# JiapengWu/TeMP

Measured on AMD Instinct MI355X. Metric: edges/sec (fwd+bwd) RGCN+GRU seq_len=15, higher is better.
Workload: dtype f32

## Files before the change

temp_amd/csrc/gemm_hx.hpp:

```cpp
#pragma once
#include "gemm_bx.hpp"
#include "hx_pack.hpp"

namespace temp {

struct HxPacked { const hx_u32x4* b[PANEL_MAXP]; const unsigned* keys[PANEL_MAXP]; };

template <int G, class Epi>
__global__ void __launch_bounds__(BX_THREADS, (G <= 4 ? 3 : 2)) k_gemm_hxp(PanelBatch<Epi> batch, BxGeom g, HxPacked packed, int keys_by_out) {
  constexpr int PIECES = G * 128;
  constexpr int NPC = (PIECES + BX_THREADS - 1) / BX_THREADS;
  __shared__ __attribute__((aligned(16))) hx_u32x4 Bs[2][PIECES];
  const PanelProblem<Epi>& pb = batch.p[blockIdx.y];
  const int M = pb.M;
  const int xcd = blockIdx.x & 7, local = blockIdx.x >> 3;
  const int grp = local % g.n_groups, rt_local = local / g.n_groups;
  const int rt = xcd * g.per_xcd + rt_local;
  if (rt_local >= g.per_xcd || rt * 128 >= M) return;
  const bool tail = grp == g.n_groups - 1;
  const int t0 = tail ? g.n_tiles - G : grp * G;
  const int t_store = tail ? G - g.tail_store : 0;
  const int n0 = t0 * 32;
  const int N = g.N, K = g.K;
  const float* __restrict__ A = pb.A;
  const int32_t* __restrict__ a_idx = pb.a_idx;
  const Epi& epi = pb.epi;
  const int lane = threadIdx.x & 63, wave = threadIdx.x >> 6;
  const int hh = lane >> 5, li = lane & 31;
  const int row = rt * 128 + wave * 32 + li;
  long a_src = -1;
  if (row < M) a_src = a_idx ? (long)a_idx[row] : (long)row;
  const float* aptr = A + (size_t)(a_src >= 0 ? a_src : 0) * g.lda;
  const unsigned akey = pb.a_keys[a_src >= 0 ? (keys_by_out ? (long)row : a_src) : 0];
  const float sa = hx_scale(akey);
  const int kclamp = K - 4;

  f32x16 acc[G];
#pragma unroll
  for (int t = 0; t < G; ++t)
#pragma unroll
    for (int r = 0; r < 16; ++r) acc[t][r] = 0.f;

  const hx_u32x4* bsrc = packed.b[blockIdx.y] + (size_t)t0 * 128;
  const size_t slab_stride = (size_t)g.n_tiles * 128;
  int piece[NPC];
#pragma unroll
  for (int i = 0; i < NPC; ++i) piece[i] = (threadIdx.x + i * BX_THREADS) % PIECES;
  hx_u32x4 br[NPC];
  const int nslabs = (K + 15) >> 4;
  auto fetch_b = [&](int s) {
    const hx_u32x4* p = bsrc + (size_t)(s < nslabs ? s : nslabs - 1) * slab_stride;
#pragma unroll
    for (int i = 0; i < NPC; ++i) br[i] = p[piece[i]];
  };
  auto fetch_a = [&](float4 (&a)[2], int k0) {
    const int k = k0 + 8 * hh;
    a[0] = ld4(aptr + (k <= kclamp ? k : kclamp));
    a[1] = ld4(aptr + (k + 4 <= kclamp ? k + 4 : kclamp));
  };
  float4 a1[2], a2[2];
  hx_u32x4 AH, AL, NH, NL;
  constexpr int NCHUNK = 4 + NPC;
  auto chunk = [&](int c, int buf) {
    if (c < 4) {
      const float4 f = a1[c >> 1];
      unsigned h, l;
      hx_split_pair((c & 1) ? f.z : f.x, (c & 1) ? f.w : f.y, sa, h, l);
      NH[c] = h; NL[c] = l;
    } else {
      Bs[buf][piece[c - 4]] = br[c - 4];
    }
  };

  fetch_b(0);
  fetch_a(a1, 0);
#pragma unroll
  for (int c = 0; c < NCHUNK; ++c) chunk(c, 0);
  AH = NH; AL = NL;
  fetch_a(a1, 16);
  __syncthreads();
  for (int s = 0; s < nslabs; ++s) {
    fetch_b(s + 1);
    fetch_a(a2, s * 16 + 32);
    const hx_f16x8 ah = hx_frag(AH), al = hx_frag(AL);
    const hx_u32x4* bs = &Bs[s & 1][lane];
    constexpr int NP = (G + 1) / 2;
    constexpr int NSLOT = (G * 3) / 2;
    constexpr int FIRST_B = NSLOT - NPC > 4 ? NSLOT - NPC : 4;
    hx_u32x4 wf[2][2][2];
#pragma unroll
    for (int u = 0; u < 2; ++u)
#pragma unroll
      for (int p = 0; p < 2; ++p)
        if (u < G) wf[0][u][p] = bs[(u * 2 + p) * 64];
    __builtin_amdgcn_sched_barrier(0);
    int slot = 0;
#pragma unroll
    for (int pr = 0; pr < NP; ++pr) {
      const bool two = 2 * pr + 1 < G;
#pragma unroll
      for (int j = 0; j < 3; ++j) {
#pragma unroll
        for (int u = 0; u < 2; ++u) {
          if (u == 1 && !two) continue;
          const int t = 2 * pr + u;
          const hx_f16x8 wh = hx_frag(wf[pr & 1][u][0]), wl = hx_frag(wf[pr & 1][u][1]);
          if (j == 0) acc[t] = __builtin_amdgcn_mfma_f32_32x32x16_f16(wl, ah, acc[t], 0, 0, 0);
          if (j == 1) acc[t] = __builtin_amdgcn_mfma_f32_32x32x16_f16(wh, al, acc[t], 0, 0, 0);
          if (j == 2) acc[t] = __builtin_amdgcn_mfma_f32_32x32x16_f16(wh, ah, acc[t], 0, 0, 0);
          if (j == 0 && pr + 1 < NP) {
            const int tn = 2 * (pr + 1) + u;
            if (tn < G) {
#pragma unroll
              for (int p = 0; p < 2; ++p) wf[(pr + 1) & 1][u][p] = bs[(tn * 2 + p) * 64];
            }
          }
          if (slot & 1) {
            const int c = slot >> 1;
            if (c < 4) chunk(c, (s + 1) & 1);
            else if (c >= FIRST_B && c - FIRST_B + 4 < NCHUNK) chunk(c - FIRST_B + 4, (s + 1) & 1);
          }
          ++slot;
          __builtin_amdgcn_sched_barrier(0);
        }
      }
    }
#pragma unroll
    for (int c = 0; c < NCHUNK; ++c) {
      const bool done = c < 4 ? c < NSLOT : (FIRST_B + c - 4 < NSLOT);
      if (!done) chunk(c, (s + 1) & 1);
    }
    a1[0] = a2[0]; a1[1] = a2[1];
    AH = NH; AL = NL;
    __syncthreads();
  }

  const bool row_ok = row < M;
  if (a_idx && a_src < 0) {
#pragma unroll
    for (int t = 0; t < G; ++t)
#pragma unroll
      for (int r = 0; r < 16; ++r) acc[t][r] = 0.f;
  }
  const typename Epi::RowCtx rc = epi.row_ctx(row_ok ? row : 0);
  const float ia = hx_inv_scale(akey);
  const unsigned* ckeys = packed.keys[blockIdx.y] + n0;
  constexpr int EG = 4;
#pragma unroll
  for (int t0e = 0; t0e < G; t0e += EG) {
    float4 pre[EG][4];
    bool ok[EG][4];
#pragma unroll
    for (int u = 0; u < EG; ++u) {
      const int t = t0e + u;
      if (t >= G) continue;
#pragma unroll
      for (int q = 0; q < 4; ++q) {
        const int col = n0 + t * 32 + 8 * q + 4 * hh;
        ok[u][q] = row_ok && col < N && t >= t_store;
        pre[u][q] = epi.pre4(rc, ok[u][q] ? row : 0, ok[u][q] ? col : 0);
      }
    }
#pragma unroll
    for (int u = 0; u < EG; ++u) {
      const int t = t0e + u;
      if (t >= G) continue;
#pragma unroll
      for (int q = 0; q < 4; ++q) {
        const int cl = t * 32 + 8 * q + 4 * hh, col = n0 + cl;
        if (ok[u][q]) {
          const float i0 = ia * hx_inv_scale(ckeys[cl]), i1 = ia * hx_inv_scale(ckeys[cl + 1]), i2 = ia * hx_inv_scale(ckeys[cl + 2]), i3 = ia * hx_inv_scale(ckeys[cl + 3]);
          epi.fin4(rc, row, col, make_float4(acc[t][4 * q] * i0, acc[t][4 * q + 1] * i1, acc[t][4 * q + 2] * i2, acc[t][4 * q + 3] * i3), pre[u][q]);
        }
      }
    }
  }
}

#define HX_KEYS_OFFSET (4u << 20)

inline size_t hx_pack_bytes(int N, int K) { return hx_packed_items(N, K) * 16 + (size_t)ceil_div(N, 32) * 32 * 4; }

static __global__ void __launch_bounds__(256) k_absmax_rows_idx(int M, int K, const float* __restrict__ A, int lda, const int32_t* __restrict__ a_idx,
                                                                unsigned* __restrict__ keys) {
  const int lane = threadIdx.x & 63, k4 = K >> 2;
  const int gw = blockIdx.x * 4 + (threadIdx.x >> 6), nw = gridDim.x * 4;
  for (int r0 = gw; r0 < M; r0 += 4 * nw) {
    float4 v[4];
    int src[4];
#pragma unroll
    for (int u = 0; u < 4; ++u) { const int r = r0 + u * nw; src[u] = r < M ? (a_idx ? a_idx[r] : r) : -1; }
#pragma unroll
    for (int u = 0; u < 4; ++u) v[u] = (src[u] >= 0 && lane < k4) ? ld4(A + (size_t)src[u] * lda + 4 * lane) : zero4();
#pragma unroll
    for (int u = 0; u < 4; ++u) {
      const int r = r0 + u * nw;
      unsigned k = hx_abs_bits4(v[u]);
      if (r < M) {
        for (int c = 256 + 4 * lane; c < K; c += 256) k = max(k, src[u] >= 0 ? hx_abs_bits4(ld4(A + (size_t)src[u] * lda + c)) : 0u);
        k = hx_wave_max(k);
        if (lane == 0) keys[r] = k;
      }
    }
  }
}

struct AbsRowsBatch { int M[PANEL_MAXP]; const float* A[PANEL_MAXP]; const int32_t* idx[PANEL_MAXP]; unsigned* keys[PANEL_MAXP]; };
static __global__ void __launch_bounds__(256) k_absmax_rows_idx_multi(AbsRowsBatch b, int K, int lda) {
  const int pr = blockIdx.y;
  const int M = b.M[pr];
  const float* __restrict__ A = b.A[pr];
  const int32_t* __restrict__ a_idx = b.idx[pr];
  unsigned* __restrict__ keys = b.keys[pr];
  const int lane = threadIdx.x & 63, k4 = K >> 2;
  const int gw = blockIdx.x * 4 + (threadIdx.x >> 6), nw = gridDim.x * 4;
  for (int r0 = gw; r0 < M; r0 += 4 * nw) {
    float4 v[4];
    int src[4];
#pragma unroll
    for (int u = 0; u < 4; ++u) { const int r = r0 + u * nw; src[u] = r < M ? (a_idx ? a_idx[r] : r) : -1; }
#pragma unroll
    for (int u = 0; u < 4; ++u) v[u] = (src[u] >= 0 && lane < k4) ? ld4(A + (size_t)src[u] * lda + 4 * lane) : zero4();
#pragma unroll
    for (int u = 0; u < 4; ++u) {
      const int r = r0 + u * nw;
      unsigned k = hx_abs_bits4(v[u]);
      if (r < M) {
        for (int c = 256 + 4 * lane; c < K; c += 256) k = max(k, src[u] >= 0 ? hx_abs_bits4(ld4(A + (size_t)src[u] * lda + c)) : 0u);
        k = hx_wave_max(k);
        if (lane == 0) keys[r] = k;
      }
    }
  }
}

template <class Epi>
static inline bool hx_supported(const PanelBatch<Epi>& batch, int count, const BxGeom& g) {
  if (!hx_enabled() || g.K % 4 || g.lda % 4) return false;
  size_t need_keys = 0;
  for (int i = 0; i < count; ++i)
    if (!batch.p[i].a_keys) need_keys += align_up((size_t)(batch.p[i].M > 0 ? batch.p[i].M : 0) * 4, 256);
  if (need_keys > 0 && ceil_div(g.N, 32) < 16 && g.K < 400 && !(option(TEMP_OPT_DEBUG) & 0x800)) return false;
  return need_keys <= BX_SLOT_BYTES - HX_KEYS_OFFSET;
}

template <class Epi>
static inline bool hx_fill_keys(PanelBatch<Epi>& batch, int count, int K, int lda, unsigned char* slot, hipStream_t st, int* keys_by_out) {
  bool any_own = false, any_given_gather = false;
  for (int i = 0; i < count; ++i) {
    if (batch.p[i].M <= 0) continue;
    if (!batch.p[i].a_keys) any_own = true;
    else if (batch.p[i].a_idx) any_given_gather = true;
  }
  if (any_own && any_given_gather) return false;
  size_t koff = HX_KEYS_OFFSET;
  AbsRowsBatch ab = {};
  int n_own = 0, max_own = 0, last = -1;
  for (int i = 0; i < count; ++i) {
    if (batch.p[i].M <= 0) { batch.p[i].a_keys = reinterpret_cast<const unsigned*>(slot + HX_KEYS_OFFSET); continue; }
    if (batch.p[i].a_keys) continue;
    unsigned* keys = reinterpret_cast<unsigned*>(slot + koff);
    koff += align_up((size_t)batch.p[i].M * 4, 256);
    ab.M[n_own] = batch.p[i].M; ab.A[n_own] = batch.p[i].A; ab.idx[n_own] = batch.p[i].a_idx; ab.keys[n_own] = keys;
    max_own = batch.p[i].M > max_own ? batch.p[i].M : max_own;
    ++n_own;
    last = i;
    batch.p[i].a_keys = keys;
  }
  if (n_own == 1) {
    int blocks = ceil_div(batch.p[last].M, 16);
    if (blocks > 2048) blocks = 2048;
    TEMP_LAUNCH(K_KEYS, k_absmax_rows_idx, dim3(blocks), dim3(256), 0, st, ab.M[0], K, ab.A[0], lda, ab.idx[0], ab.keys[0]);
  } else if (n_own > 1) {
    int blocks = ceil_div(max_own, 16);
    if (blocks > 2048 / n_own) blocks = 2048 / n_own;
    TEMP_LAUNCH(K_KEYS, k_absmax_rows_idx_multi, dim3(blocks, n_own), dim3(256), 0, st, ab, K, lda);
  }
  for (int i = count; i < PANEL_MAXP; ++i) batch.p[i].a_keys = batch.p[0].a_keys;
  *keys_by_out = any_own ? 1 : 0;
  return true;
}

template <int G, class Epi>
static inline void launch_hxp_g(int kid, const PanelBatch<Epi>& batch, int count, const BxGeom& g, hipStream_t st, const HxPacked& pk, int keys_by_out) {
  dim3 grid(8 * g.per_xcd * g.n_groups, count);
  gemm_route_count(TEMP_ROUTE_HXP, G);
  TEMP_LAUNCH(kid, (k_gemm_hxp<G, Epi>), grid, dim3(BX_THREADS), 0, st, batch, g, pk, keys_by_out);
}

template <class Epi>
int launch_gemm_hx(int kid, const PanelBatch<Epi>& batch_in, int count, const BxGeom& g, int G, hipStream_t st) {
  const size_t pbytes = align_up(hx_pack_bytes(g.N, g.K), 256);
  int n_distinct = 0, which[PANEL_MAXP];
  for (int i = 0; i < count; ++i) {
    which[i] = -1;
    for (int j = 0; j < i; ++j)
      if (batch_in.p[j].B == batch_in.p[i].B) { which[i] = which[j]; break; }
    if (which[i] < 0) which[i] = n_distinct++;
  }
  if (pbytes * n_distinct > BX_PACK_MAX_BYTES || n_distinct > HX_PACK_JOBS) return TEMP_E_UNSUPPORTED;
  unsigned char* slot = reinterpret_cast<unsigned char*>(bx_scratch(st, BX_SLOT_BYTES));
  if (!slot) return TEMP_E_UNSUPPORTED;
  PanelBatch<Epi> batch = batch_in;
  HxPacked pk;
  HxPackJobs jobs = {};
  const size_t items = hx_packed_items(g.N, g.K);
  int done = 0;
  for (int i = 0; i < PANEL_MAXP; ++i) { pk.b[i] = reinterpret_cast<const hx_u32x4*>(slot); pk.keys[i] = reinterpret_cast<const unsigned*>(slot + items * 16); }
  for (int i = 0; i < count; ++i) {
    unsigned char* dst = slot + (size_t)which[i] * pbytes;
    pk.b[i] = reinterpret_cast<const hx_u32x4*>(dst);
    pk.keys[i] = reinterpret_cast<const unsigned*>(dst + items * 16);
    if (which[i] < done) continue;
    ++done;
    hx_pack_jobs_add(jobs, batch.p[i].B, reinterpret_cast<hx_u32x4*>(dst), reinterpret_cast<unsigned*>(dst + items * 16), g.K, g.N, g.ldb, g.trans_b);
  }
  int kbo = 0;
  if (!hx_fill_keys(batch, count, g.K, g.lda, slot, st, &kbo)) return TEMP_E_UNSUPPORTED;
  hx_pack_launch(jobs, K_BX_PACK, st);
  hx_count();
  switch (G) {
    case 1: launch_hxp_g<1, Epi>(kid, batch, count, g, st, pk, kbo); break;
    case 2: launch_hxp_g<2, Epi>(kid, batch, count, g, st, pk, kbo); break;
    case 3: launch_hxp_g<3, Epi>(kid, batch, count, g, st, pk, kbo); break;
    case 4: launch_hxp_g<4, Epi>(kid, batch, count, g, st, pk, kbo); break;
    case 5: launch_hxp_g<5, Epi>(kid, batch, count, g, st, pk, kbo); break;
    case 6: launch_hxp_g<6, Epi>(kid, batch, count, g, st, pk, kbo); break;
    default: launch_hxp_g<7, Epi>(kid, batch, count, g, st, pk, kbo); break;
  }
  return launch_status();
}

}
#include "gemm_hxr.hpp"
namespace temp {

template <class Epi>
static inline bool launch_hxr(int kid, const PanelBatch<Epi>& batch_in, int count, const BxGeom& g, hipStream_t st) {
  if (!option(TEMP_OPT_GEMM_RESIDENT) || g.K > BXR_MAX_SLABS * 16 || g.K < 72 || g.K % 8 || !hx_supported(batch_in, count, g)) return false;
  int max_m = 0;
  for (int i = 0; i < count; ++i) max_m = batch_in.p[i].M > max_m ? batch_in.p[i].M : max_m;
  BxrGeom rg;
  if (!bxr_plan(g.N, g.K, g.lda, max_m, &rg)) return false;
  rg.ldb = g.ldb; rg.trans_b = g.trans_b;
  static const bool granted = hipFuncSetAttribute(reinterpret_cast<const void*>(k_gemm_hxr<Epi>), hipFuncAttributeMaxDynamicSharedMemorySize, HXR_LDS_BYTES) == hipSuccess;
  if (!granted) { (void)hipGetLastError(); return false; }
  PanelBatch<Epi> batch = batch_in;
  bool need = false;
  for (int i = 0; i < count; ++i) need = need || (batch.p[i].M > 0 && !batch.p[i].a_keys);
  int kbo = 0;
  if (need) {
    unsigned char* slot = reinterpret_cast<unsigned char*>(bx_scratch(st, BX_SLOT_BYTES));
    if (!slot || !hx_fill_keys(batch, count, g.K, g.lda, slot, st, &kbo)) return false;
  } else {
    for (int i = 0; i < PANEL_MAXP; ++i) if (!batch.p[i].a_keys) batch.p[i].a_keys = batch.p[0].a_keys;
    for (int i = 0; i < count; ++i) if (batch.p[i].M > 0) { for (int j = 0; j < PANEL_MAXP; ++j) if (!batch.p[j].a_keys) batch.p[j].a_keys = batch.p[i].a_keys; break; }
  }
  const size_t lds = (size_t)rg.n_slabs * BXR_G * 128 * 16 + 3 * BXR_BIAS_BYTES;
  gemm_route_count(TEMP_ROUTE_HXR, 0);
  TEMP_LAUNCH(kid, (k_gemm_hxr<Epi>), dim3(256, count), dim3(BXR_WAVES * 64), lds, st, batch, rg, kbo);
  hx_count();
  return true;
}

}
```

Measured before the change: 954.7 million.

## Add 4-deep A-register ring pipeline and LDS-staged column inverse scales in hx GEMM

Replaces the main loop of the split-fp16 panel GEMM with a ring of four A-register prefetch buffers fully unrolled by four, so A loads for slab s+4 are issued early while MFMAs run on the current slab. B fragments are double-buffered across tile pairs, and byte offsets for B pieces are precomputed. The epilogue now computes column inverse scales once into shared memory and reads them as float4 instead of recomputing per element from global keys. This adds register pressure and code size, and keeps the old path behind a debug flag; VAR template variants for probing are unused by default.

```diff
diff --git a/temp_amd/csrc/gemm_hx.hpp b/temp_amd/csrc/gemm_hx.hpp
--- a/temp_amd/csrc/gemm_hx.hpp
+++ b/temp_amd/csrc/gemm_hx.hpp
@@ -1,12 +1,14 @@
 #pragma once
 #include "gemm_bx.hpp"
 #include "hx_pack.hpp"
+#include <type_traits>
 
 namespace temp {
 
 struct HxPacked { const hx_u32x4* b[PANEL_MAXP]; const unsigned* keys[PANEL_MAXP]; };
 
-template <int G, class Epi>
+#define HXP_OLD_BODY 0x1000000
+template <int G, class Epi, bool RING = true, int VAR = 0>
 __global__ void __launch_bounds__(BX_THREADS, (G <= 4 ? 3 : 2)) k_gemm_hxp(PanelBatch<Epi> batch, BxGeom g, HxPacked packed, int keys_by_out) {
   constexpr int PIECES = G * 128;
   constexpr int NPC = (PIECES + BX_THREADS - 1) / BX_THREADS;
@@ -33,6 +35,7 @@
   const float* aptr = A + (size_t)(a_src >= 0 ? a_src : 0) * g.lda;
   const unsigned akey = pb.a_keys[a_src >= 0 ? (keys_by_out ? (long)row : a_src) : 0];
   const float sa = hx_scale(akey);
+  const bool zero_row = a_idx && a_src < 0;
   const int kclamp = K - 4;
 
   f32x16 acc[G];
@@ -55,9 +58,131 @@
   };
   auto fetch_a = [&](float4 (&a)[2], int k0) {
     const int k = k0 + 8 * hh;
+    if constexpr (VAR & 1) { a[0] = make_float4(1.f, 2.f, 3.f, (float)k0); a[1] = a[0]; return; }
     a[0] = ld4(aptr + (k <= kclamp ? k : kclamp));
     a[1] = ld4(aptr + (k + 4 <= kclamp ? k + 4 : kclamp));
   };
+  unsigned ckey_own = 0;
+  if constexpr (RING) ckey_own = packed.keys[blockIdx.y][n0 + (threadIdx.x < G * 32 ? (int)threadIdx.x : 0)];
+  if constexpr (RING) {
+    constexpr int NCHUNK = 4 + NPC;
+    constexpr int NP = (G + 1) / 2;
+    constexpr int NSLOT = (G * 3) / 2;
+    constexpr int FIRST_B = NSLOT - NPC > 4 ? NSLOT - NPC : 4;
+    float4 R[4][2];
+    hx_u32x4 F[2][2];
+    unsigned pbyte[NPC];
+#pragma unroll
+    for (int i = 0; i < NPC; ++i) pbyte[i] = (unsigned)piece[i] * 16u;
+    auto fetch_b = [&](int s) {
+      const char* p = reinterpret_cast<const char*>(bsrc + (size_t)(s < nslabs ? s : nslabs - 1) * slab_stride);
+#pragma unroll
+      for (int i = 0; i < NPC; ++i) br[i] = *reinterpret_cast<const hx_u32x4*>(p + pbyte[i]);
+    };
+    auto store_b = [&](int buf, int i) { *reinterpret_cast<hx_u32x4*>(reinterpret_cast<char*>(&Bs[buf][0]) + pbyte[i]) = br[i]; };
+    fetch_b(0);
+    __builtin_amdgcn_sched_barrier(0);
+#pragma unroll
+    for (int j = 0; j < 4; ++j) fetch_a(R[j], 16 * j);
+#pragma unroll
+    for (int c = 0; c < 4; ++c) {
+      const float4 f = R[0][c >> 1];
+      unsigned h, l;
+      hx_split_pair((c & 1) ? f.z : f.x, (c & 1) ? f.w : f.y, sa, h, l);
+      F[0][0][c] = h; F[0][1][c] = l;
+    }
+#pragma unroll
+    for (int i = 0; i < NPC; ++i) store_b(0, i);
+    __syncthreads();
+    auto body = [&](auto jc, int s) __attribute__((always_inline)) {
+      constexpr int j = decltype(jc)::value;
+      asm volatile("" : "+s"(s));
+      float sab = sa;
+      asm volatile("" : "+v"(sab));
+      fetch_b(s + 1);
+      __builtin_amdgcn_sched_barrier(0);
+      fetch_a(R[j], s * 16 + 64);
+      hx_u32x4 (&CF)[2] = F[j & 1];
+      hx_u32x4 (&NF)[2] = F[(j + 1) & 1];
+      const float4 (&rn)[2] = R[(j + 1) & 3];
+      auto chunk = [&](int c) {
+        if (c < 4) {
+          const float4 f = rn[c >> 1];
+          unsigned h, l;
+          hx_split_pair((c & 1) ? f.z : f.x, (c & 1) ? f.w : f.y, sab, h, l);
+          NF[0][c] = h; NF[1][c] = l;
+        } else {
+          store_b((j + 1) & 1, c - 4);
+        }
+      };
+      const hx_f16x8 ah = hx_frag(CF[0]), al = hx_frag(CF[1]);
+      const hx_u32x4* bs = &Bs[j & 1][lane];
+      hx_u32x4 wf[2][2][2];
+#pragma unroll
+      for (int u = 0; u < 2; ++u)
+#pragma unroll
+        for (int p = 0; p < 2; ++p)
+          if (u < G) wf[0][u][p] = bs[(u * 2 + p) * 64];
+      __builtin_amdgcn_sched_barrier(0);
+      int slot = 0;
+#pragma unroll
+      for (int pr = 0; pr < NP; ++pr) {
+        const bool two = 2 * pr + 1 < G;
+#pragma unroll
+        for (int jj = 0; jj < 3; ++jj) {
+#pragma unroll
+          for (int u = 0; u < 2; ++u) {
+            if (u == 1 && !two) continue;
+            const int t = 2 * pr + u;
+            const hx_f16x8 wh = hx_frag(wf[pr & 1][u][0]), wl = hx_frag(wf[pr & 1][u][1]);
+            if constexpr (!(VAR & 4)) {
+              if (jj == 0) acc[t] = __builtin_amdgcn_mfma_f32_32x32x16_f16(wl, ah, acc[t], 0, 0, 0);
+              if (jj == 1) acc[t] = __builtin_amdgcn_mfma_f32_32x32x16_f16(wh, al, acc[t], 0, 0, 0);
+              if (jj == 2) acc[t] = __builtin_amdgcn_mfma_f32_32x32x16_f16(wh, ah, acc[t], 0, 0, 0);
+            } else if (jj == 0) {
+              acc[t][0] += __builtin_bit_cast(float, wf[pr & 1][u][0][0] ^ wf[pr & 1][u][1][1] ^ CF[0][0] ^ CF[1][1]);
+            }
+            if (jj == 0 && pr + 1 < NP) {
+              const int tn = 2 * (pr + 1) + u;
+              if (tn < G) {
+#pragma unroll
+                for (int p = 0; p < 2; ++p) wf[(pr + 1) & 1][u][p] = bs[(tn * 2 + p) * 64];
+              }
+            }
+            if (slot & 1) {
+              const int c = slot >> 1;
+              if (c < 4) chunk(c);
+              else if (c >= FIRST_B && c - FIRST_B + 4 < NCHUNK) chunk(c - FIRST_B + 4);
+            }
+            ++slot;
+            __builtin_amdgcn_sched_barrier(0);
+          }
+        }
+      }
+#pragma unroll
+      for (int c = 0; c < NCHUNK; ++c) {
+        const bool done = c < 4 ? c < NSLOT : (FIRST_B + c - 4 < NSLOT);
+        if (!done) chunk(c);
+      }
+      asm volatile("" : "+v"(NF[0]), "+v"(NF[1]));
+      __syncthreads();
+    };
+    using std::integral_constant;
+    int s = 0;
+    for (; s + 4 <= nslabs; s += 4) {
+      body(integral_constant<int, 0>(), s);
+      body(integral_constant<int, 1>(), s + 1);
+      body(integral_constant<int, 2>(), s + 2);
+      body(integral_constant<int, 3>(), s + 3);
+    }
+    if (s < nslabs) {
+      body(integral_constant<int, 0>(), s);
+      if (s + 1 < nslabs) {
+        body(integral_constant<int, 1>(), s + 1);
+        if (s + 2 < nslabs) body(integral_constant<int, 2>(), s + 2);
+      }
+    }
+  } else {
   float4 a1[2], a2[2];
   hx_u32x4 AH, AL, NH, NL;
   constexpr int NCHUNK = 4 + NPC;
@@ -134,9 +259,10 @@
     AH = NH; AL = NL;
     __syncthreads();
   }
+  }
 
   const bool row_ok = row < M;
-  if (a_idx && a_src < 0) {
+  if (zero_row) {
 #pragma unroll
     for (int t = 0; t < G; ++t)
 #pragma unroll
@@ -144,8 +270,46 @@
   }
   const typename Epi::RowCtx rc = epi.row_ctx(row_ok ? row : 0);
   const float ia = hx_inv_scale(akey);
+  constexpr int EG = 4;
+  if constexpr (RING) {
+    float* cinv = reinterpret_cast<float*>(&Bs[0][0]);
+    if (threadIdx.x < G * 32) cinv[threadIdx.x] = hx_inv_scale(ckey_own);
+    __syncthreads();
+    const Epi e = epi;
+#pragma unroll
+    for (int t0e = 0; t0e < G; t0e += EG) {
+      float4 pre[EG][4];
+      bool ok[EG][4];
+#pragma unroll
+      for (int u = 0; u < EG; ++u) {
+        const int t = t0e + u;
+        if (t >= G) continue;
+#pragma unroll
+        for (int q = 0; q < 4; ++q) {
+          const int col = n0 + t * 32 + 8 * q + 4 * hh;
+          ok[u][q] = row_ok && col < N && t >= t_store;
+          pre[u][q] = e.pre4(rc, ok[u][q] ? row : 0, ok[u][q] ? col : 0);
+        }
+      }
+#pragma unroll
+      for (int u = 0; u < EG; ++u) {
+        const int t = t0e + u;
+        if (t >= G) continue;
+        float4 cis[4];
+#pragma unroll
+        for (int q = 0; q < 4; ++q) cis[q] = *reinterpret_cast<const float4*>(cinv + t * 32 + 8 * q + 4 * hh);
+#pragma unroll
+        for (int q = 0; q < 4; ++q) {
+          const int col = n0 + t * 32 + 8 * q + 4 * hh;
+          const float4 ci = cis[q];
+          if constexpr (VAR & 2) { if (acc[t][4 * q] == 12345.678f) e.fin4(rc, row, col, zero4(), pre[u][q]); continue; }
+          if (ok[u][q])
+            e.fin4(rc, row, col, make_float4(acc[t][4 * q] * (ia * ci.x), acc[t][4 * q + 1] * (ia * ci.y), acc[t][4 * q + 2] * (ia * ci.z), acc[t][4 * q + 3] * (ia * ci.w)), pre[u][q]);
+        }
+      }
+    }
+  } else {
   const unsigned* ckeys = packed.keys[blockIdx.y] + n0;
-  constexpr int EG = 4;
 #pragma unroll
   for (int t0e = 0; t0e < G; t0e += EG) {
     float4 pre[EG][4];
@@ -174,6 +338,7 @@
         }
       }
     }
+  }
   }
 }
 
@@ -285,6 +450,7 @@
 static inline void launch_hxp_g(int kid, const PanelBatch<Epi>& batch, int count, const BxGeom& g, hipStream_t st, const HxPacked& pk, int keys_by_out) {
   dim3 grid(8 * g.per_xcd * g.n_groups, count);
   gemm_route_count(TEMP_ROUTE_HXP, G);
+  if (option(TEMP_OPT_DEBUG) & HXP_OLD_BODY) { TEMP_LAUNCH(kid, (k_gemm_hxp<G, Epi, false>), grid, dim3(BX_THREADS), 0, st, batch, g, pk, keys_by_out); return; }
   TEMP_LAUNCH(kid, (k_gemm_hxp<G, Epi>), grid, dim3(BX_THREADS), 0, st, batch, g, pk, keys_by_out);
 }
 
```

Result: no change. 956.1 million (median of 2 runs) (+0.1%).
